# facebookresearch/detectron2

Hardware: NVIDIA H100
Metric: Mask R-CNN R50-FPN training hot-path images/sec (custom-op path fwd+bwd, 2 images/GPU) (higher is better)
Workload: dtype f32

## Files before the change

### detectron2_b200/csrc/deform_conv_tc.cu

```cuda
#include <algorithm>
#include <cstdlib>
#include <type_traits>

#include "common.cuh"
#include "deform_conv_tc.cuh"
#include "tc_common.cuh"

using namespace d2b_tc;

namespace {

constexpr int kWorkerWarps = 16;
constexpr int kWorkers = kWorkerWarps * 32;
constexpr int kThreads = kWorkers + 128;
constexpr int kLaunchRegs = (65536 / kThreads) & ~7;
constexpr int kWorkerRegs = 112, kSideRegs = 24;
static_assert(kWorkers * kWorkerRegs + (kThreads - kWorkers) * kSideRegs <= kThreads * kLaunchRegs,
              "register budget exceeds the launch allocation");
constexpr int kSideRegsMax = ((kThreads * kLaunchRegs - kWorkers * kWorkerRegs) / (kThreads - kWorkers)) & ~7;
static_assert(kSideRegsMax >= kSideRegs, "register budget exceeds the launch allocation");
constexpr int kMaxBN = 128;
constexpr int kRowsPerHalf = 128 / (2 * kWorkerWarps);
constexpr int kTile = 16384;
constexpr int kMaxSmem = 227 * 1024;
// ... 9 lines not shown
  long long off_bs, mask_bs;
  int mask_sigmoid;
};

struct Epi {
  const float* scale;
  const float* shift;
  int relu;
};

struct K1P { int BN, noct, goct, uper, ksplit, S, tap_bytes, stage_bytes, red; };
struct K2P { int mper, msplit, tap_bytes; };
struct K3P { int BN, noct, sper, nsplit, S, stage_bytes; };

inline size_t align256(size_t v) { return (v + 255) & ~(size_t)255; }

bool make_tc(const d2b_dcn_params* p, TC& d) {
  if (!p) return false;
  d.N = p->N; d.Cin = p->Cin; d.H = p->H; d.W = p->W; d.Cout = p->Cout; d.kh = p->kh; d.kw = p->kw;
  d.sh = p->stride_h; d.sw = p->stride_w; d.ph = p->pad_h; d.pw = p->pad_w; d.dh = p->dil_h; d.dw = p->dil_w;
  d.G = p->groups; d.DG = p->deformable_groups;
  if (d.N < 0 || d.Cin <= 0 || d.H <= 0 || d.W <= 0 || d.Cout <= 0 || d.kh <= 0 || d.kw <= 0 || d.sh <= 0 || d.sw <= 0 ||
      d.ph < 0 || d.pw < 0 || d.dh <= 0 || d.dw <= 0 || d.G <= 0 || d.DG <= 0)
    return false;
  if (d.Cin % d.G || d.Cout % d.G || d.Cin % d.DG) return false;
  d.Ho = (d.H + 2 * d.ph - (d.dh * (d.kh - 1) + 1)) / d.sh + 1;
  d.Wo = (d.W + 2 * d.pw - (d.dw * (d.kw - 1) + 1)) / d.sw + 1;
  if (d.Ho <= 0 || d.Wo <= 0) return false;
  d.cpg = d.Cin / d.G; d.opg = d.Cout / d.G; d.cpdg = d.Cin / d.DG; d.KK = d.kh * d.kw; d.HoWo = d.Ho * d.Wo;
  if (d.cpg >= 64) {
    if (d.cpg % 64) return false;
    d.pack = 1;
  } else {
    if (d.cpg != 16 && d.cpg != 32) return false;
    d.pack = 64 / d.cpg;
    if (d.G % d.pack) return false;
  }
  if (d.cpdg % 64) return false;
  d.SG = d.G / d.pack; d.cps = d.cpg * d.pack; d.ops = d.opg * d.pack; d.cbs = d.cps / 64; d.U = d.KK * d.cbs;
  if (d.ops % 16) return false;
  if (d.KK > 49) return false;
  if ((long long)d.H * d.W * d.Cin >= (1LL << 29)) return false;
  if ((long long)d.HoWo * d.Cout >= (1LL << 31) || (long long)d.Cout * d.cpg * d.KK >= (1LL << 31)) return false;
  d.tiles_img = d2b_cdiv(d.HoWo, 128);
  d.stages_img = d2b_cdiv(d.HoWo, 64);
  d.MC = (d.U + 1) / 2;
  d.nks = d.ops / 64;
  if ((long long)d.N * d.tiles_img > 0x7fffffffLL) return false;
  d.off_bs = (long long)d.DG * 2 * d.KK * d.HoWo;
  d.mask_bs = (long long)d.DG * d.KK * d.HoWo;
  d.mask_sigmoid = 0;
  return true;
}

const float* use_fused_offset_mask(TC& d, const float* offset_mask) {
  d.off_bs = d.mask_bs = (long long)d.DG * 3 * d.KK * d.HoWo;
  d.mask_sigmoid = 1;
  return offset_mask + (size_t)d.DG * 2 * d.KK * d.HoWo;
}

int largest_tile(int n) {
  for (int t = kMaxBN; t >= 16; t >>= 1)
    if (n % t == 0) return t;
  return 0;
}

int best_split(long long base, int work, int max_split, int overhead) {
  int best = 1;
  long long best_cost = -1;
  for (int s = 1; s <= max_split; ++s) {
    const int per = d2b_cdiv(work, s);
    const int parts = d2b_cdiv(work, per);
    const long long cost = (long long)d2b_cdiv(base * parts, d2b_num_sms()) * (per + overhead);
    if (best_cost < 0 || cost < best_cost) {
      best_cost = cost;
      best = parts;
    }
  }
  return best;
}

int k1_tap_points(const TC& d, int units) { return std::min(d.KK, (units + d.cbs - 2) / d.cbs + 1); }

bool plan_k1(const TC& d, K1P& k, bool colfed = false) {
  k.BN = largest_tile(d.ops);
  if (k.BN < 16) return false;
  k.noct = d.ops / k.BN;
  k.goct = colfed ? 1 : k.noct;
  const int base = d.N * d.tiles_img * d.SG * k.goct;
  k.ksplit = best_split(base, d.U, d.U, d.cbs);
  k.uper = d2b_cdiv(d.U, k.ksplit);
  k.ksplit = d2b_cdiv(d.U, k.uper);
  k.red = k.ksplit > 1;
  const int ndg = d.DG == 1 ? 1 : std::min(d.DG, d2b_cdiv(d.cps, d.cpdg) + 1);
  k.tap_bytes = ndg * k1_tap_points(d, k.uper) * 128 * 16;
  k.stage_bytes = 2 * kTile + 2 * k.BN * 128;
  k.S = 3;
  while (k.S > 1 && k.S * k.stage_bytes + k.tap_bytes + 1024 + 128 > kMaxSmem) --k.S;
  return k.S >= 2;
}

bool plan_k1c(const TC& d, K1P& k1, K1P& kc) {
  const long long base = (long long)d.N * d.tiles_img * d.SG * (k1.noct - 1);
  if (k1.goct != 1 || k1.noct < 2 || (long long)d.N * d.tiles_img * (k1.noct - 1) > 0x7fffffffLL) return false;
  kc = k1;
  kc.goct = k1.noct - 1;
  kc.ksplit = best_split(base, d.U, d.U, d.cbs);
  kc.uper = d2b_cdiv(d.U, kc.ksplit);
  kc.ksplit = d2b_cdiv(d.U, kc.uper);
  kc.tap_bytes = 0;
  kc.S = 3;
  while (kc.S > 1 && kc.S * kc.stage_bytes + 1024 + 128 > kMaxSmem) --kc.S;
  if (kc.S < 2) return false;
  k1.red = kc.red = k1.ksplit > 1 || kc.ksplit > 1;
  return true;
}

bool plan_k2(const TC& d, K2P& k) {
  if (d.ops % 64) return false;
  const int base = d.N * d.tiles_img * d.SG;
  k.msplit = best_split(base, d.MC, d.MC, 1);
  k.mper = d2b_cdiv(d.MC, k.msplit);
  k.msplit = d2b_cdiv(d.MC, k.mper);
  const int nkp = std::min(d.KK, (2 * k.mper + d.cbs - 1) / d.cbs + 1);
  const int ndg = d.DG == 1 ? 1 : std::min(d.DG, d2b_cdiv(d.cps, d.cpdg) + 1);
  k.tap_bytes = ndg * nkp * 128 * 16;
  return 2 * 4 * kTile + 128 * kGcolPitch * 4 + k.tap_bytes + 1024 + 128 <= kMaxSmem;
}

bool plan_k3(const TC& d, K3P& k) {
  if (d.ops % 64) return false;
  k.BN = largest_tile(d.ops);
  k.noct = d.ops / k.BN;
  const int units = d.MC * d.SG * k.noct;
  const int total = d.N * d.stages_img;
  k.nsplit = best_split(units, total, std::min(total, 4 * d2b_num_sms()), 3);
  k.sper = d2b_cdiv(total, k.nsplit);
  k.nsplit = d2b_cdiv(total, k.sper);
  k.stage_bytes = 2 * kTile + 2 * k.BN * 128;
  k.S = 3;
  while (k.S > 1 && k.S * k.stage_bytes + 4096 + 1024 + 128 > kMaxSmem) --k.S;
  return k.S >= 2;
}

struct Carve {
  size_t total = 0;
  size_t add(size_t bytes) {
    const size_t at = total;
    total += align256(bytes);
    return at;
  }
};

struct FwdPlan {
  TC d;
  K1P k1, kc;
  bool colfed;
  int split;
  size_t wt, x, total;
  size_t cols_bytes;
};

bool plan_fwd(const d2b_dcn_params* p, int precision, int x_nhwc, bool cols, FwdPlan& P) {
  if (!make_tc(p, P.d) || !plan_k1(P.d, P.k1)) return false;
  const TC& d = P.d;
  Carve ws;
  P.wt = ws.add((size_t)d.SG * P.k1.noct * d.U * 2 * P.k1.BN * 128);
  P.x = ws.add(x_nhwc ? 0 : sizeof(float) * (size_t)d.N * d.H * d.W * d.Cin);
  P.total = ws.total;
  P.cols_bytes = (size_t)d.N * d.tiles_img * d.SG * d.U * (size_t)(precision == 1 ? 2 : 1) * kTile;
  P.split = precision == 1 ? 1 : 0;
  P.colfed = false;
  K1P k1;
  if (cols && P.k1.noct > 1 && plan_k1(d, k1, true) && plan_k1c(d, k1, P.kc)) {
    P.k1 = k1;
    P.colfed = true;
  }
  return true;
}

struct BwdPlan {
  TC d;
  K2P k2;
  K3P k3;
  int split;
  size_t x, gx, gt_px, wt, gt_oc, gw, gw_bytes, total;
};

bool plan_bwd(const d2b_dcn_params* p, int precision, int x_nhwc, int need_data, int need_weight, BwdPlan& P) {
  if (!make_tc(p, P.d) || !plan_k2(P.d, P.k2) || !plan_k3(P.d, P.k3)) return false;
  const TC& d = P.d;
  const size_t xbytes = sizeof(float) * (size_t)d.N * d.H * d.W * d.Cin;
  P.gw_bytes = sizeof(float) * (size_t)d.SG * d.MC * 128 * d.ops;
  Carve ws;
  P.x = ws.add(x_nhwc ? 0 : xbytes);
  P.gx = ws.add(need_data && !x_nhwc ? xbytes : 0);
  P.gt_px = ws.add(need_data ? (size_t)d.N * d.tiles_img * d.SG * d.nks * 2 * kTile : 0);
  P.wt = ws.add(need_data ? (size_t)d.SG * d.MC * d.nks * 2 * kTile : 0);
  P.gt_oc = ws.add(need_weight ? (size_t)d.N * d.stages_img * d.SG * P.k3.noct * 2 * P.k3.BN * 128 : 0);
  P.gw = ws.add(need_weight ? P.gw_bytes : 0);
  P.total = ws.total;
  P.split = precision == 1 ? 1 : 0;
  return true;
}

struct TapRaw {
  float oh, ow, m;
};

__device__ __forceinline__ TapRaw tap_loads(const TC& d, const float* __restrict__ offset, const float* __restrict__ mask,
                                            int b, int dg, int kp, int p) {
  TapRaw r = {0.f, 0.f, 1.f};
  if (p < d.HoWo) {
    const size_t ob = (size_t)b * d.off_bs + ((size_t)dg * 2 * d.KK) * d.HoWo;
    r.oh = __ldg(offset + ob + (size_t)(2 * kp) * d.HoWo + p);
    r.ow = __ldg(offset + ob + (size_t)(2 * kp + 1) * d.HoWo + p);
    if (mask) r.m = __ldg(mask + (size_t)b * d.mask_bs + ((size_t)dg * d.KK + kp) * d.HoWo + p);
  }
  return r;
}

__device__ __forceinline__ int4 tap_finish(const TC& d, const TapRaw& r, bool has_mask, int kp, int p) {
  int4 t = make_int4(0, 0, 0, 0);
  if (p < d.HoWo) {
    const int ho = p / d.Wo, wo = p - ho * d.Wo;
    const int ki = kp / d.kw, kj = kp - ki * d.kw;
    const float hf = (float)(ho * d.sh - d.ph + ki * d.dh) + r.oh;
    const float wf = (float)(wo * d.sw - d.pw + kj * d.dw) + r.ow;
    float m = r.m;
    if (has_mask && d.mask_sigmoid) m = 1.f / (1.f + expf(-m));
    if (hf > -1.f && wf > -1.f && hf < (float)d.H && wf < (float)d.W) {
      const float hfl = floorf(hf), wfl = floorf(wf);
      const int hl = (int)hfl, wl = (int)wfl;
      const bool t0 = hl >= 0, t1 = hl + 1 <= d.H - 1, l0 = wl >= 0, l1 = wl + 1 <= d.W - 1;
      const int flags = (t0 && l0 ? 1 : 0) | (t0 && l1 ? 2 : 0) | (t1 && l0 ? 4 : 0) | (t1 && l1 ? 8 : 0);
      t.x = ((hl * d.W + wl + d.W + 1) << 4) | flags;
      t.y = __float_as_int(hf - hfl);
      t.z = __float_as_int(wf - wfl);
      t.w = __float_as_int(m);
    }
  }
  return t;
}

__device__ __forceinline__ int4 make_tap(const TC& d, const float* __restrict__ offset, const float* __restrict__ mask,
                                         int b, int dg, int kp, int p) {
  return tap_finish(d, tap_loads(d, offset, mask, b, dg, kp, p), mask != nullptr, kp, p);
}

struct Taps4 {
  float4 v0, v1, v2, v3;
};

__device__ __forceinline__ void load_corners(const float* __restrict__ xcb, uint32_t Cin, uint32_t rs, int code, Taps4& t) {
  const float* __restrict__ p = xcb + (uint32_t)(code >> 4) * Cin;
  const float4 z = make_float4(0.f, 0.f, 0.f, 0.f);
  t.v0 = (code & 1) ? __ldg(reinterpret_cast<const float4*>(p)) : z;
  t.v1 = (code & 2) ? __ldg(reinterpret_cast<const float4*>(p + Cin)) : z;
  t.v2 = (code & 4) ? __ldg(reinterpret_cast<const float4*>(p + rs)) : z;
  t.v3 = (code & 8) ? __ldg(reinterpret_cast<const float4*>(p + (rs + Cin))) : z;
}

__device__ __forceinline__ void interp4(const Taps4& t, float w0, float w1, float w2, float w3, float (&v)[4]) {
  const F2 z = f2_pack(0.f, 0.f), p0 = f2_pack(w0, w0), p1 = f2_pack(w1, w1), p2 = f2_pack(w2, w2), p3 = f2_pack(w3, w3);
  F2 a = f2_fma(p0, f2_pack(t.v0.x, t.v0.y), z), b = f2_fma(p0, f2_pack(t.v0.z, t.v0.w), z);
  a = f2_fma(p1, f2_pack(t.v1.x, t.v1.y), a);
  b = f2_fma(p1, f2_pack(t.v1.z, t.v1.w), b);
  a = f2_fma(p2, f2_pack(t.v2.x, t.v2.y), a);
  b = f2_fma(p2, f2_pack(t.v2.z, t.v2.w), b);
  a = f2_fma(p3, f2_pack(t.v3.x, t.v3.y), a);
  b = f2_fma(p3, f2_pack(t.v3.z, t.v3.w), b);
  f2_unpack(a, v[0], v[1]);
  f2_unpack(b, v[2], v[3]);
}

__device__ __forceinline__ void gather_store(const Taps4& t, int4 tap, uint8_t* a_hi, uint8_t* a_lo, uint32_t off,
                                             bool split) {
  const float lh = __int_as_float(tap.y), lw = __int_as_float(tap.z), m = __int_as_float(tap.w);
  const float hh = 1.f - lh, hw = 1.f - lw;
  float v[4];
  interp4(t, hh * hw * m, hh * lw * m, lh * hw * m, lh * lw * m, v);
  uint2 hi, lo;
  split4(v, hi, lo);
  *reinterpret_cast<uint2*>(a_hi + off) = hi;
  if (split) *reinterpret_cast<uint2*>(a_lo + off) = lo;
}

template <int BN, int kTransA, int kSplit>
__device__ __forceinline__ void mma_stage_(float (&acc)[BN / 4], uint32_t a_hi, uint32_t a_lo, uint32_t b_hi, uint32_t b_lo) {
  const int g = (threadIdx.x >> 7);
  const uint32_t ao = kTransA ? (uint32_t)(g & 1) * 8192u : (uint32_t)(g & 1) * 64u * 128u;
  const uint32_t bo = (uint32_t)(g >> 1) * (uint32_t)(BN / 2) * 128u;
  const uint32_t lbo = kTransA ? 8192u : 0u;
  wgmma_fence();
#pragma unroll
  for (int kk = 0; kk < 4; ++kk) {
    const uint32_t ak = ao + (kTransA ? (uint32_t)kk * 2048u : (uint32_t)kk * 32u), bk = bo + (uint32_t)kk * 32u;
    Wgmma<BN / 2, kTransA>::mma(acc, wgmma_desc(a_hi + ak, lbo, 1024), wgmma_desc(b_hi + bk, 0, 1024), 1);
    if (kSplit) {
      Wgmma<BN / 2, kTransA>::mma(acc, wgmma_desc(a_hi + ak, lbo, 1024), wgmma_desc(b_lo + bk, 0, 1024), 1);
      Wgmma<BN / 2, kTransA>::mma(acc, wgmma_desc(a_lo + ak, lbo, 1024), wgmma_desc(b_hi + bk, 0, 1024), 1);
    }
  }
  wgmma_commit();
}
template <int BN, int kTransA>
__device__ __forceinline__ void mma_stage(float (&acc)[BN / 4], uint32_t a_hi, uint32_t a_lo, uint32_t b_hi, uint32_t b_lo,
                                          int split) {
  if (split) mma_stage_<BN, kTransA, 1>(acc, a_hi, a_lo, b_hi, b_lo);
  else mma_stage_<BN, kTransA, 0>(acc, a_hi, a_lo, b_hi, b_lo);
}

template <int BN>
__device__ __forceinline__ int acc_row(int i) {
  const int t = threadIdx.x & 127;
  return (threadIdx.x >> 7 & 1) * 64 + (t >> 5) * 16 + ((t & 31) >> 2) + ((i >> 1) & 1) * 8;
}
template <int BN>
__device__ __forceinline__ int acc_col(int i) {
  return (threadIdx.x >> 8) * (BN / 2) + (i >> 2) * 8 + (threadIdx.x & 3) * 2 + (i & 1);
}

template <int BN>
__device__ __forceinline__ void fwd_epilogue(const float (&acc)[BN / 4], const Epi& ep, const TC& d, const K1P& k,
                                             float* __restrict__ out, int b, int p0, int oc0) {
  const bool add_shift = ep.shift != nullptr && blockIdx.z == 0;
#pragma unroll
  for (int i = 0; i < BN / 4; ++i) {
    const int p = p0 + acc_row<BN>(i);
    if (p >= d.HoWo) continue;
    const int oc = oc0 + acc_col<BN>(i);
    float* dst = out + ((size_t)b * d.Cout + oc) * d.HoWo + p;
    float v = acc[i];
    if (k.red) {
      red_add(dst, v + ((add_shift && !ep.scale && !ep.relu) ? __ldg(ep.shift + oc) : 0.f));
    } else {
      if (ep.scale) v *= __ldg(ep.scale + oc);
      if (ep.shift) v += __ldg(ep.shift + oc);
      if (ep.relu) v = fmaxf(v, 0.f);
      *dst = v;
    }
  }
}

template <int BN>
__global__ void __launch_bounds__(kThreads, 1) dcn_fwd_tc_kernel(const float* __restrict__ xh,
                                                                   const float* __restrict__ offset,
                                                                   const float* __restrict__ mask,
                                                                   const uint8_t* __restrict__ wt, const Epi ep, const TC d,
                                                                   const K1P k, const int split, float* __restrict__ out,
                                                                   uint8_t* __restrict__ cols) {
// ... 548 lines not shown
      if (have_next && lane < 2 * PX)
        my_taps[((i + 1) & 1) * (2 * PX) + lane] =
            tl_ok ? tap_finish(d, raw, mask != nullptr, tl_kp, pbn + warp * PX + tl_j) : make_int4(0, 0, 0, 0);
      fence_proxy_async();
      __syncwarp();
      if (lane == 0) mbar_arrive(&full_bar[s]);
      mbar_wait(&full_bar[s], par);
      const uint32_t sa = smem_u32(smem + s * k.stage_bytes), sb = sa + 2 * kTile;
      mma_stage<BN, 1>(acc, sa, sa + kTile, sb, sb + (uint32_t)BN * 128u, split);
    };
    stage(0);
    for (int i = 1; i < ns; ++i) {
      stage(i);
      wgmma_wait<1>();
      __syncwarp();
      if (lane == 0) mbar_arrive(&empty_bar[(i - 1) % k.S]);
    }
    wgmma_wait<0>();
    gw_tile_store<BN>(acc, gw + ((size_t)sg * d.MC * 128 + (size_t)mb * 128) * d.ops + (size_t)oct * k.BN, d.ops);
  } else if (warp == kWorkerWarps) {
    if (lane == 0) {
      const uint32_t bytes = (uint32_t)(split ? 2 : 1) * (uint32_t)k.BN * 128u;
      for (int i = 0; i < ns; ++i) {
        const int s = i % k.S;
        const uint32_t par = (uint32_t)((i / k.S) & 1);
        mbar_wait(&empty_bar[s], par ^ 1u);
        mbar_arrive_expect_tx(&full_bar[s], bytes);
        const size_t tile = ((size_t)(gs0 + i) * d.SG + sg) * k.noct + oct;
        bulk_g2s(smem + s * k.stage_bytes + 2 * kTile, gt + tile * (size_t)(2 * k.BN * 128), bytes, &full_bar[s]);
      }
    }
  }
}

template <int BN, int kSide>
__device__ __forceinline__ void bwd_weight_cols_body(uint8_t* smem, int bx, int by, int bz, const uint8_t* __restrict__ cols,
                                                     const uint8_t* __restrict__ gt, const TC& d, const K3P& k, const int S,
                                                     const int split, float* __restrict__ gw) {
  uint64_t* bars = reinterpret_cast<uint64_t*>(smem + S * k.stage_bytes);
  uint64_t* full_bar = bars;
  uint64_t* empty_bar = bars + S;

  const int tid = threadIdx.x, warp = tid >> 5, lane = tid & 31;
  const int mb = by;
  const int sg = bx / k.noct, oct = bx - sg * k.noct;
  const int total = d.N * d.stages_img;
  const int gs0 = bz * k.sper, gs1 = min(total, gs0 + k.sper), ns = gs1 - gs0;
  const int nu = (2 * mb + 1 < d.U) ? 2 : 1;

  if (tid == 0) {
    for (int s = 0; s < S; ++s) {
      mbar_init(&full_bar[s], 1);
      mbar_init(&empty_bar[s], kWorkerWarps);
    }
    mbar_init_fence();
  }
  if (nu == 1 && tid < kWorkers) {
    for (int s = 0; s < S; ++s)
      for (int i = tid; i < 2 * 512; i += kWorkers) {
        const int part = i >> 9, w = i & 511;
        reinterpret_cast<uint4*>(smem + s * k.stage_bytes + part * kTile + 8192)[w] = make_uint4(0, 0, 0, 0);
      }
    fence_proxy_async();
  }
  __syncthreads();
  if (warp < kWorkerWarps) reg_alloc<kWorkerRegs>();
  else reg_dealloc<kSide>();

  if (warp < kWorkerWarps) {
    float acc[BN / 4];
#pragma unroll
    for (int i = 0; i < BN / 4; ++i) acc[i] = 0.f;
    auto issue = [&](int i) {
      const int s = i % S;
      mbar_wait(&full_bar[s], (uint32_t)((i / S) & 1));
      const uint32_t sa = smem_u32(smem + s * k.stage_bytes), sb = sa + 2 * kTile;
      mma_stage<BN, 1>(acc, sa, sa + kTile, sb, sb + (uint32_t)BN * 128u, split);
    };
    issue(0);
    for (int i = 1; i < ns; ++i) {
      issue(i);
      wgmma_wait<1>();
      __syncwarp();
      if (lane == 0) mbar_arrive(&empty_bar[(i - 1) % S]);
    }
    wgmma_wait<0>();
    gw_tile_store<BN>(acc, gw + ((size_t)sg * d.MC * 128 + (size_t)mb * 128) * d.ops + (size_t)oct * k.BN, d.ops);
  } else if (warp == kWorkerWarps) {
    if (lane == 0) {
      const uint32_t parts = split ? 2u : 1u;
      const uint32_t tile_bytes = parts * (uint32_t)kTile;
      const uint32_t gbytes = parts * (uint32_t)k.BN * 128u;
      for (int i = 0; i < ns; ++i) {
        const int s = i % S;
        const uint32_t par = (uint32_t)((i / S) & 1);
        const int gs = gs0 + i;
        const int b = gs / d.stages_img, st = gs - b * d.stages_img;
        mbar_wait(&empty_bar[s], par ^ 1u);
        mbar_arrive_expect_tx(&full_bar[s], (uint32_t)nu * parts * 8192u + gbytes);
        uint8_t* stage = smem + s * k.stage_bytes;
        const uint8_t* src =
            cols + ((((size_t)b * d.tiles_img + (st >> 1)) * d.SG + sg) * d.U + 2 * mb) * tile_bytes + (size_t)(st & 1) * 8192;
        for (int ul = 0; ul < nu; ++ul)
          for (uint32_t part = 0; part < parts; ++part)
            bulk_g2s(stage + part * kTile + ul * 8192, src + (size_t)ul * tile_bytes + (size_t)part * kTile, 8192u, &full_bar[s]);
        const size_t tile = ((size_t)gs * d.SG + sg) * k.noct + oct;
        bulk_g2s(stage + 2 * kTile, gt + tile * (size_t)(2 * k.BN * 128), gbytes, &full_bar[s]);
      }
    }
  }
}

template <int BN>
__global__ void __launch_bounds__(kThreads, 1) dcn_bwd_weight_cols_kernel(const uint8_t* __restrict__ cols,
                                                                          const uint8_t* __restrict__ gt, const TC d,
                                                                          const K3P k, const int S, const int split,
                                                                          float* __restrict__ gw) {
  bwd_weight_cols_body<BN, kSideRegs>(aligned_smem(), blockIdx.x, blockIdx.y, blockIdx.z, cols, gt, d, k, S, split, gw);
}

template <int BN>
__global__ void __launch_bounds__(kThreads, 1) dcn_bwd_fused_kernel(const float* __restrict__ xh,
                                                                    const float* __restrict__ offset,
                                                                    const float* __restrict__ mask,
                                                                    const uint8_t* __restrict__ gt_px,
                                                                    const uint8_t* __restrict__ wt, const K2P k2,
                                                                    float* __restrict__ gxh, float* __restrict__ goff,
                                                                    float* __restrict__ gmask,
                                                                    const uint8_t* __restrict__ cols,
                                                                    const uint8_t* __restrict__ gt_oc, const K3P k3,
                                                                    const int S3, float* __restrict__ gw, const TC d,
                                                                    const int split) {
  const int nx2 = d.N * d.tiles_img, n2 = nx2 * d.SG * k2.msplit;
  int id = blockIdx.x;
  if (id < n2) {
    const int bx = id % nx2, r = id / nx2;
    bwd_data_body<kSideRegsMax>(aligned_smem(), bx, r % d.SG, r / d.SG, xh, offset, mask, gt_px, wt, d, k2, split, gxh, goff,
                                gmask);
  } else {
    id -= n2;
    const int nx3 = d.SG * k3.noct, r = id / nx3;
    bwd_weight_cols_body<BN, kSideRegsMax>(aligned_smem(), id % nx3, r % d.MC, r / d.MC, cols, gt_oc, d, k3, S3, split,
                                           gw);
  }
}

__device__ __forceinline__ void split8(const float (&v)[8], uint4& hi, uint4& lo) {
  split2(v[0], v[1], hi.x, lo.x);
  split2(v[2], v[3], hi.y, lo.y);
  split2(v[4], v[5], hi.z, lo.z);
  split2(v[6], v[7], hi.w, lo.w);
}

__device__ __forceinline__ float w_elem(const float* __restrict__ w, const TC& d, int oc, int c, int kp) {
  const int g = c / d.cpg;
  if (oc / d.opg != g) return 0.f;
  return __ldg(w + ((size_t)oc * d.cpg + (c - g * d.cpg)) * d.KK + kp);
}

__global__ void dcn_wtile_fwd_kernel(const float* __restrict__ w, const TC d, int BN, int noct, uint8_t* __restrict__ dst) {
  const long long idx = (long long)blockIdx.x * blockDim.x + threadIdx.x;
  const long long total = (long long)d.SG * noct * d.U * BN * 8;
  if (idx >= total) return;
  const int c16 = (int)(idx & 7);
  const int r = (int)((idx >> 3) % BN);
  const long long tile = idx / (8LL * BN);
  const int u = (int)(tile % d.U);
  const int oct = (int)((tile / d.U) % noct);
  const int sg = (int)(tile / ((long long)d.U * noct));
  const int kp = u / d.cbs, cb = u - kp * d.cbs;
  const int oc = sg * d.ops + oct * BN + r;
  float v[8];
#pragma unroll
  for (int e = 0; e < 8; ++e) v[e] = w_elem(w, d, oc, sg * d.cps + cb * 64 + c16 * 8 + e, kp);
  uint4 hi, lo;
  split8(v, hi, lo);
  uint8_t* base = dst + tile * (size_t)(2 * BN * 128);
  *reinterpret_cast<uint4*>(base + swz128((uint32_t)r, (uint32_t)c16)) = hi;
  *reinterpret_cast<uint4*>(base + BN * 128 + swz128((uint32_t)r, (uint32_t)c16)) = lo;
}

__global__ void dcn_wtile_bwd_kernel(const float* __restrict__ w, const TC d, uint8_t* __restrict__ dst) {
  const long long idx = (long long)blockIdx.x * blockDim.x + threadIdx.x;
  const long long total = (long long)d.SG * d.MC * d.nks * 128 * 8;
  if (idx >= total) return;
  const int c16 = (int)(idx & 7);
  const int r = (int)((idx >> 3) & 127);
  const long long tile = idx >> 10;
  const int ks = (int)(tile % d.nks);
  const int m = (int)((tile / d.nks) % d.MC);
  const int sg = (int)(tile / ((long long)d.nks * d.MC));
  const int u = 2 * m + (r >> 6);
  float v[8];
#pragma unroll
  for (int e = 0; e < 8; ++e) v[e] = 0.f;
  if (u < d.U) {
    const int kp = u / d.cbs, cb = u - kp * d.cbs;
    const int c = sg * d.cps + cb * 64 + (r & 63);
#pragma unroll
    for (int e = 0; e < 8; ++e) v[e] = w_elem(w, d, sg * d.ops + ks * 64 + c16 * 8 + e, c, kp);
  }
  uint4 hi, lo;
  split8(v, hi, lo);
  uint8_t* base = dst + tile * (size_t)(2 * kTile);
  *reinterpret_cast<uint4*>(base + swz128((uint32_t)r, (uint32_t)c16)) = hi;
  *reinterpret_cast<uint4*>(base + kTile + swz128((uint32_t)r, (uint32_t)c16)) = lo;
}

__device__ __forceinline__ float gout_elem(const float* __restrict__ gout, const float* __restrict__ ysaved, const Epi& ep,
                                           size_t idx, int oc) {
  float g = __ldg(gout + idx);
  if (ep.relu && !(__ldg(ysaved + idx) > 0.f)) g = 0.f;
  if (ep.scale) g *= __ldg(ep.scale + oc);
  return g;
}

__global__ void __launch_bounds__(256) dcn_gout_px_tiles_kernel(const float* __restrict__ gout,
                                                                const float* __restrict__ ysaved, const Epi ep, const TC d,
                                                                uint8_t* __restrict__ dst, uint8_t* __restrict__ dst_oc,
                                                                int BN, int noct) {
  __shared__ float t[64][33];
  const long long tile = blockIdx.x;
  const int ks = (int)(tile % d.nks);
  const int sg = (int)((tile / d.nks) % d.SG);
  const int pt = (int)((tile / ((long long)d.nks * d.SG)) % d.tiles_img);
  const int b = (int)(tile / ((long long)d.nks * d.SG * d.tiles_img));
  const int r0 = blockIdx.y * 32;
  const int p0 = pt * 128 + r0, oc0 = sg * d.ops + ks * 64;
  const int tid = threadIdx.x;
#pragma unroll
  for (int i = 0; i < 8; ++i) {
    const int e = tid + i * 256;
    const int o = e >> 5, pp = e & 31;
    const int p = p0 + pp;
    t[o][pp] = p < d.HoWo ? gout_elem(gout, ysaved, ep, ((size_t)b * d.Cout + oc0 + o) * d.HoWo + p, oc0 + o) : 0.f;
  }
  __syncthreads();
  uint8_t* base = dst + tile * (size_t)(2 * kTile);
  {
    const int r = tid >> 3, c16 = tid & 7;
    float v[8];
#pragma unroll
    for (int i = 0; i < 8; ++i) v[i] = t[c16 * 8 + i][r];
    uint4 hi, lo;
    split8(v, hi, lo);
    *reinterpret_cast<uint4*>(base + swz128((uint32_t)(r0 + r), (uint32_t)c16)) = hi;
    *reinterpret_cast<uint4*>(base + kTile + swz128((uint32_t)(r0 + r), (uint32_t)c16)) = lo;
  }
  if (dst_oc) {
    const int o = tid >> 2, ch = tid & 3;
    const int ocs = ks * 64 + o;
    const int oct = ocs / BN, row = ocs - oct * BN;
    const int pglob = pt * 128 + r0;
    const int ps = pglob >> 6, c16 = ((pglob & 63) >> 3) + ch;
    float v[8];
#pragma unroll
    for (int i = 0; i < 8; ++i) v[i] = t[o][ch * 8 + i];
    uint4 hi, lo;
    split8(v, hi, lo);
    if (ps < d.stages_img) {
      const size_t tile_oc = (((size_t)b * d.stages_img + ps) * d.SG + sg) * noct + oct;
      uint8_t* bo = dst_oc + tile_oc * (size_t)(2 * BN * 128);
      *reinterpret_cast<uint4*>(bo + swz128((uint32_t)row, (uint32_t)c16)) = hi;
      *reinterpret_cast<uint4*>(bo + BN * 128 + swz128((uint32_t)row, (uint32_t)c16)) = lo;
    }
  }
}

__global__ void dcn_gout_oc_tiles_kernel(const float* __restrict__ gout, const float* __restrict__ ysaved, const Epi ep,
                                         const TC d, int BN, int noct, uint8_t* __restrict__ dst) {
  const long long idx = (long long)blockIdx.x * blockDim.x + threadIdx.x;
  const long long total = (long long)d.N * d.stages_img * d.SG * noct * BN * 8;
  if (idx >= total) return;
  const int c16 = (int)(idx & 7);
  const int r = (int)((idx >> 3) % BN);
  const long long tile = idx / (8LL * BN);
  const int oct = (int)(tile % noct);
  const int sg = (int)((tile / noct) % d.SG);
  const int ps = (int)((tile / ((long long)noct * d.SG)) % d.stages_img);
  const int b = (int)(tile / ((long long)noct * d.SG * d.stages_img));
  const int oc = sg * d.ops + oct * BN + r;
  const size_t src = ((size_t)b * d.Cout + oc) * d.HoWo;
  float v[8];
#pragma unroll
  for (int e = 0; e < 8; ++e) {
    const int p = ps * 64 + c16 * 8 + e;
    v[e] = p < d.HoWo ? gout_elem(gout, ysaved, ep, src + p, oc) : 0.f;
  }
  uint4 hi, lo;
  split8(v, hi, lo);
  uint8_t* base = dst + tile * (size_t)(2 * BN * 128);
  *reinterpret_cast<uint4*>(base + swz128((uint32_t)r, (uint32_t)c16)) = hi;
  *reinterpret_cast<uint4*>(base + BN * 128 + swz128((uint32_t)r, (uint32_t)c16)) = lo;
}

__global__ void dcn_epilogue_kernel(float* __restrict__ y, long long total, int Cout, int HoWo, const Epi ep) {
  const long long i = (long long)blockIdx.x * blockDim.x + threadIdx.x;
  if (i >= total) return;
  const int oc = (int)((i / HoWo) % Cout);
  float v = y[i];
  if (ep.scale) v *= __ldg(ep.scale + oc);
  if (ep.shift) v += __ldg(ep.shift + oc);
  if (ep.relu) v = fmaxf(v, 0.f);
  y[i] = v;
}

int change_layout(const float* src, const TC& d, float* dst, bool to_nhwc, cudaStream_t stream) {
  d2b_pyramid P = {};
  P.num_levels = 1;
  P.feat[0] = src;
  P.H[0] = d.H;
  P.W[0] = d.W;
  P.scale[0] = 1.f;
  float* dsts[1] = {dst};
  return to_nhwc ? d2b_pyramid_nchw_to_nhwc(&P, d.N, d.Cin, dsts, D2B_F32, (void*)stream)
                 : d2b_pyramid_nhwc_to_nchw(&P, d.N, d.Cin, reinterpret_cast<void* const*>(dsts), D2B_F32, (void*)stream);
}

template <auto kernel, class... Args>
int launch_big_smem(dim3 grid, int smem_bytes, cudaStream_t stream, Args... args) {
  D2B_ALLOW_BIG_SMEM(kernel);
  kernel<<<grid, kThreads, smem_bytes, stream>>>(args...);
  D2B_CHECK_LAUNCH();
  return D2B_OK;
}

template <int W, int... More, class Launch>
int with_tile_width(int BN, Launch launch) {
  if constexpr (sizeof...(More) > 0)
    if (BN != W) return with_tile_width<More...>(BN, launch);
  return launch(std::integral_constant<int, W>());
}

}

D2B_API int d2b_deform_conv_tc_shape_supported(const d2b_dcn_params* p, int backward) {
  FwdPlan f;
  BwdPlan b;
  return backward ? plan_bwd(p, 1, 1, 1, 1, b) : plan_fwd(p, 1, 1, false, f);
}

size_t d2b_deform_conv_tc_fwd_workspace(const d2b_dcn_params* p, int precision, int x_nhwc) {
  FwdPlan P;
  return plan_fwd(p, precision, x_nhwc, false, P) ? P.total : 0;
}

size_t d2b_deform_conv_tc_bwd_workspace(const d2b_dcn_params* p, int precision, int x_nhwc, int need_data, int need_weight) {
  BwdPlan P;
  return plan_bwd(p, precision, x_nhwc, need_data, need_weight, P) ? P.total : 0;
}

size_t d2b_deform_conv_tc_cols_bytes(const d2b_dcn_params* p, int precision) {
  FwdPlan f;
  BwdPlan b;
  return plan_fwd(p, precision, 1, false, f) && plan_bwd(p, precision, 1, 0, 0, b) ? f.cols_bytes : 0;
}

int d2b_deform_conv_forward_tc(const float* x, const float* offset, const float* mask, const float* weight,
                               const float* scale, const float* shift, int relu, const d2b_dcn_params* p, int precision,
                               int tcflags, float* out, void* cols, void* workspace, size_t workspace_bytes, void* stream_) {
  cudaStream_t stream = (cudaStream_t)stream_;
  const int x_nhwc = tcflags & 1;
  FwdPlan P;
  if (!plan_fwd(p, precision, x_nhwc, cols != nullptr, P)) return D2B_EUNSUPPORTED;
  TC& d = P.d;
  const K1P& k = P.k1;
  if (d.N == 0) return D2B_OK;
  if (tcflags & 2) {
    if (mask) return D2B_EINVAL;
    mask = use_fused_offset_mask(d, offset);
  }
  if (!workspace || workspace_bytes < P.total) return D2B_EWORKSPACE;
  if ((reinterpret_cast<uintptr_t>(workspace) & 255) || (x_nhwc && (reinterpret_cast<uintptr_t>(x) & 15)) ||
      (reinterpret_cast<uintptr_t>(cols) & 15))
    return D2B_EINVAL;
  uint8_t* ws = reinterpret_cast<uint8_t*>(workspace);
  uint8_t* wt = ws + P.wt;
  const float* xh = x;
  if (!x_nhwc) {
    float* xn = reinterpret_cast<float*>(ws + P.x);
    if (int rc = change_layout(x, d, xn, true, stream)) return rc;
    xh = xn;
  }
  {
    const long long total = (long long)d.SG * k.noct * d.U * k.BN * 8;
    dcn_wtile_fwd_kernel<<<d2b_cdiv(total, 256), 256, 0, stream>>>(weight, d, k.BN, k.noct, wt);
    D2B_CHECK_LAUNCH();
  }
  if (k.red) D2B_CUDA(cudaMemsetAsync(out, 0, sizeof(float) * (size_t)d.N * d.Cout * d.HoWo, stream));
  const Epi ep = {scale, shift, relu};
  const dim3 grid(d.N * d.tiles_img, d.SG * k.goct, k.ksplit);
  const int smem_bytes = k.S * k.stage_bytes + k.tap_bytes + 1024 + 128;
  int rc = with_tile_width<16, 32, 64, 128>(k.BN, [&](auto bn) {
    return launch_big_smem<dcn_fwd_tc_kernel<decltype(bn)::value>>(grid, smem_bytes, stream, xh, offset, mask, wt, ep, d, k,
                                                                    P.split, out, reinterpret_cast<uint8_t*>(cols));
  });
  if (rc) return rc;
  if (P.colfed) {
    const K1P& kc = P.kc;
    const dim3 grid_c(d.N * d.tiles_img * kc.goct, d.SG, kc.ksplit);
    const int smem_c = kc.S * kc.stage_bytes + 1024 + 128;
    const uint8_t* cl = reinterpret_cast<const uint8_t*>(cols);
    rc = with_tile_width<16, 32, 64, 128>(kc.BN, [&](auto bn) {
      return launch_big_smem<dcn_fwd_cols_kernel<decltype(bn)::value>>(grid_c, smem_c, stream, cl, wt, ep, d, kc, P.split,
                                                                        out);
    });
    if (rc) return rc;
  }
  if (k.red && (scale || relu)) {
    const long long total = (long long)d.N * d.Cout * d.HoWo;
    dcn_epilogue_kernel<<<d2b_cdiv(total, 256), 256, 0, stream>>>(out, total, d.Cout, d.HoWo, ep);
    D2B_CHECK_LAUNCH();
  }
  return D2B_OK;
}

int d2b_deform_conv_backward_tc(const float* x, const float* offset, const float* mask, const float* weight,
                                const float* grad_out, const float* scale, const float* y_saved, int relu,
                                const d2b_dcn_params* p, int precision, int tcflags, const void* cols, float* grad_x,
                                float* grad_offset, float* grad_mask, float* grad_weight, void* workspace,
                                size_t workspace_bytes, void* stream_) {
  cudaStream_t stream = (cudaStream_t)stream_;
  const int x_nhwc = tcflags & 1;
  const int need_data = (grad_x || grad_offset || grad_mask) ? 1 : 0, need_weight = grad_weight ? 1 : 0;
  BwdPlan P;
  if (!plan_bwd(p, precision, x_nhwc, need_data, need_weight, P)) return D2B_EUNSUPPORTED;
  TC& d = P.d;
  const K2P& k2 = P.k2;
  const K3P& k3 = P.k3;
  const bool fused_om = (tcflags & 2) != 0;
  if (fused_om && (mask || grad_mask)) return D2B_EINVAL;
  if (relu && !y_saved) return D2B_EINVAL;
  const size_t nx = (size_t)d.N * d.H * d.W * d.Cin, noff = (size_t)d.N * d.DG * (fused_om ? 3 : 2) * d.KK * d.HoWo;
  const size_t nm = (size_t)d.N * d.DG * d.KK * d.HoWo, nw = (size_t)d.Cout * d.cpg * d.KK;
  if (fused_om) {
    mask = use_fused_offset_mask(d, offset);
    if (grad_offset) grad_mask = grad_offset + (size_t)d.DG * 2 * d.KK * d.HoWo;
  }
  const Epi ep = {scale, nullptr, relu};
  if (d.N == 0 || (!need_data && !need_weight)) {
    void* zp[3] = {grad_offset, fused_om ? nullptr : grad_mask, grad_weight};
    size_t zb[3] = {noff * 4, nm * 4, nw * 4};
    return d2b_zero_buffers(zp, zb, 3, stream);
  }
  if (!workspace || workspace_bytes < P.total) return D2B_EWORKSPACE;
  if ((reinterpret_cast<uintptr_t>(workspace) & 255) || (x_nhwc && (reinterpret_cast<uintptr_t>(x) & 15)) ||
      (x_nhwc && grad_x && (reinterpret_cast<uintptr_t>(grad_x) & 15)) || (reinterpret_cast<uintptr_t>(cols) & 15))
    return D2B_EINVAL;
  uint8_t* ws = reinterpret_cast<uint8_t*>(workspace);
  const float* xh = x;
  if (!x_nhwc) {
    float* xn = reinterpret_cast<float*>(ws + P.x);
    if (int rc = change_layout(x, d, xn, true, stream)) return rc;
    xh = xn;
  }
  float* gxh = grad_x ? (x_nhwc ? grad_x : reinterpret_cast<float*>(ws + P.gx)) : nullptr;
  uint8_t* gt_oc = need_weight ? ws + P.gt_oc : nullptr;
  float* gw_part = need_weight ? reinterpret_cast<float*>(ws + P.gw) : nullptr;
  {
    void* zp[4] = {grad_offset, fused_om ? nullptr : grad_mask, gxh, gw_part};
    size_t zb[4] = {noff * 4, nm * 4, nx * 4, P.gw_bytes};
    int rc = d2b_zero_buffers(zp, zb, 4, stream);
    if (rc) return rc;
  }
  const long long fused_ctas = (long long)d.N * d.tiles_img * d.SG * k2.msplit + (long long)d.SG * k3.noct * d.MC * k3.nsplit;
  const bool fused = need_data && need_weight && cols && fused_ctas <= 0x7fffffffLL;
  const uint8_t* cl = reinterpret_cast<const uint8_t*>(cols);
  const int S3 = std::min(6, (kMaxSmem - 2048) / k3.stage_bytes);
  const int smem3 = S3 * k3.stage_bytes + 1024 + 128;
  if (need_data) {
    uint8_t* gt_px = ws + P.gt_px;
    uint8_t* wt = ws + P.wt;
    dcn_gout_px_tiles_kernel<<<dim3((unsigned)((size_t)d.N * d.tiles_img * d.SG * d.nks), 4), 256, 0, stream>>>(
        grad_out, y_saved, ep, d, gt_px, gt_oc, k3.BN, k3.noct);
    D2B_CHECK_LAUNCH();
    {
      const long long total = (long long)d.SG * d.MC * d.nks * 128 * 8;
      dcn_wtile_bwd_kernel<<<d2b_cdiv(total, 256), 256, 0, stream>>>(weight, d, wt);
      D2B_CHECK_LAUNCH();
    }
    const int smem2 = 2 * 4 * kTile + 128 * kGcolPitch * 4 + k2.tap_bytes + 1024 + 128;
    float* gm = mask ? grad_mask : nullptr;
    int rc;
    if (fused) {
      rc = with_tile_width<64, 128>(k3.BN, [&](auto bn) {
        return launch_big_smem<dcn_bwd_fused_kernel<decltype(bn)::value>>(
            dim3((unsigned)fused_ctas), std::max(smem2, smem3), stream, xh, offset, mask, gt_px, wt, k2, gxh, grad_offset, gm,
            cl, gt_oc, k3, S3, gw_part, d, P.split);
      });
    } else {
      rc = launch_big_smem<dcn_bwd_data_tc_kernel>(dim3(d.N * d.tiles_img, d.SG, k2.msplit), smem2, stream, xh, offset, mask,
                                                   gt_px, wt, d, k2, P.split, gxh, grad_offset, gm);
    }
    if (rc) return rc;
    if (grad_x && !x_nhwc) {
      if (int rc = change_layout(gxh, d, grad_x, false, stream)) return rc;
    }
  }
  if (need_weight) {
    if (!need_data) {
      const long long total = (long long)d.N * d.stages_img * d.SG * k3.noct * k3.BN * 8;
      dcn_gout_oc_tiles_kernel<<<d2b_cdiv(total, 256), 256, 0, stream>>>(grad_out, y_saved, ep, d, k3.BN, k3.noct, gt_oc);
      D2B_CHECK_LAUNCH();
    }
    if (!fused) {
      const dim3 grid(d.SG * k3.noct, d.MC, k3.nsplit);
      int rc;
      if (cols) {
        rc = with_tile_width<64, 128>(k3.BN, [&](auto bn) {
          return launch_big_smem<dcn_bwd_weight_cols_kernel<decltype(bn)::value>>(grid, smem3, stream, cl, gt_oc, d, k3, S3,
                                                                                   P.split, gw_part);
        });
      } else {
        const int smem_bytes = k3.S * k3.stage_bytes + 4096 + 1024 + 128;
        rc = with_tile_width<64, 128>(k3.BN, [&](auto bn) {
          return launch_big_smem<dcn_bwd_weight_tc_kernel<decltype(bn)::value>>(grid, smem_bytes, stream, xh, offset, mask,
                                                                                 gt_oc, d, k3, P.split, gw_part);
        });
      }
      if (rc) return rc;
    }
    if (d.KK <= 9) {
      dcn_gw_reduce_tile_kernel<<<dim3(d.SG * (d.cps / kRedCh), d.ops / kRedOc), 256, 0, stream>>>(gw_part, d, grad_weight);
    } else {
      const long long total = (long long)d.SG * d.U * 64 * d.ops;
      dcn_gw_reduce_kernel<<<d2b_cdiv(total, 256), 256, 0, stream>>>(gw_part, d, grad_weight);
    }
    D2B_CHECK_LAUNCH();
  }
  return D2B_OK;
}
```

Baseline: 300.3.

## Build fwd and bwd DCN weight tiles in one smem-staged kernel, reuse in backward

Replaces the two per-element weight-tiling kernels with one kernel that stages a block of weights in shared memory using vectorized loads and writes both forward and backward swizzled tiles. The backward tile is stored after the saved columns buffer during forward, so backward skips rebuilding it when columns are available. This cuts global-load redundancy and one launch per backward, at the cost of a larger saved columns buffer. It also assumes ops divisible by 16/64 and KK<=49, which can break for other shapes.

```diff
diff --git a/detectron2_b200/csrc/deform_conv_tc.cu b/detectron2_b200/csrc/deform_conv_tc.cu
--- a/detectron2_b200/csrc/deform_conv_tc.cu
+++ b/detectron2_b200/csrc/deform_conv_tc.cu
@@ -185,13 +185,18 @@
   }
 };
 
+size_t wt_bwd_bytes(const TC& d) { return (size_t)d.SG * d.MC * d.nks * 2 * kTile; }
+size_t cols_wt_offset(const TC& d, int precision) {
+  return ((size_t)d.N * d.tiles_img * d.SG * d.U * (size_t)(precision == 1 ? 2 : 1) * kTile + 1023) & ~(size_t)1023;
+}
+
 struct FwdPlan {
   TC d;
   K1P k1, kc;
   bool colfed;
   int split;
   size_t wt, x, total;
-  size_t cols_bytes;
+  size_t cols_wt, cols_bytes;
 };
 
 bool plan_fwd(const d2b_dcn_params* p, int precision, int x_nhwc, bool cols, FwdPlan& P) {
@@ -201,7 +206,8 @@
   P.wt = ws.add((size_t)d.SG * P.k1.noct * d.U * 2 * P.k1.BN * 128);
   P.x = ws.add(x_nhwc ? 0 : sizeof(float) * (size_t)d.N * d.H * d.W * d.Cin);
   P.total = ws.total;
-  P.cols_bytes = (size_t)d.N * d.tiles_img * d.SG * d.U * (size_t)(precision == 1 ? 2 : 1) * kTile;
+  P.cols_wt = cols_wt_offset(d, precision);
+  P.cols_bytes = P.cols_wt + (d.ops % 64 == 0 ? wt_bwd_bytes(d) : 0);
   P.split = precision == 1 ? 1 : 0;
   P.colfed = false;
   K1P k1;
@@ -229,7 +235,7 @@
   P.x = ws.add(x_nhwc ? 0 : xbytes);
   P.gx = ws.add(need_data && !x_nhwc ? xbytes : 0);
   P.gt_px = ws.add(need_data ? (size_t)d.N * d.tiles_img * d.SG * d.nks * 2 * kTile : 0);
-  P.wt = ws.add(need_data ? (size_t)d.SG * d.MC * d.nks * 2 * kTile : 0);
+  P.wt = ws.add(need_data ? wt_bwd_bytes(d) : 0);
   P.gt_oc = ws.add(need_weight ? (size_t)d.N * d.stages_img * d.SG * P.k3.noct * 2 * P.k3.BN * 128 : 0);
   P.gw = ws.add(need_weight ? P.gw_bytes : 0);
   P.total = ws.total;
@@ -1084,59 +1090,83 @@
   split2(v[6], v[7], hi.w, lo.w);
 }
 
-__device__ __forceinline__ float w_elem(const float* __restrict__ w, const TC& d, int oc, int c, int kp) {
-  const int g = c / d.cpg;
-  if (oc / d.opg != g) return 0.f;
-  return __ldg(w + ((size_t)oc * d.cpg + (c - g * d.cpg)) * d.KK + kp);
-}
-
-__global__ void dcn_wtile_fwd_kernel(const float* __restrict__ w, const TC d, int BN, int noct, uint8_t* __restrict__ dst) {
-  const long long idx = (long long)blockIdx.x * blockDim.x + threadIdx.x;
-  const long long total = (long long)d.SG * noct * d.U * BN * 8;
-  if (idx >= total) return;
-  const int c16 = (int)(idx & 7);
-  const int r = (int)((idx >> 3) % BN);
-  const long long tile = idx / (8LL * BN);
-  const int u = (int)(tile % d.U);
-  const int oct = (int)((tile / d.U) % noct);
-  const int sg = (int)(tile / ((long long)d.U * noct));
-  const int kp = u / d.cbs, cb = u - kp * d.cbs;
-  const int oc = sg * d.ops + oct * BN + r;
-  float v[8];
-#pragma unroll
-  for (int e = 0; e < 8; ++e) v[e] = w_elem(w, d, oc, sg * d.cps + cb * 64 + c16 * 8 + e, kp);
-  uint4 hi, lo;
-  split8(v, hi, lo);
-  uint8_t* base = dst + tile * (size_t)(2 * BN * 128);
-  *reinterpret_cast<uint4*>(base + swz128((uint32_t)r, (uint32_t)c16)) = hi;
-  *reinterpret_cast<uint4*>(base + BN * 128 + swz128((uint32_t)r, (uint32_t)c16)) = lo;
-}
-
-__global__ void dcn_wtile_bwd_kernel(const float* __restrict__ w, const TC d, uint8_t* __restrict__ dst) {
-  const long long idx = (long long)blockIdx.x * blockDim.x + threadIdx.x;
-  const long long total = (long long)d.SG * d.MC * d.nks * 128 * 8;
-  if (idx >= total) return;
-  const int c16 = (int)(idx & 7);
-  const int r = (int)((idx >> 3) & 127);
-  const long long tile = idx >> 10;
-  const int ks = (int)(tile % d.nks);
-  const int m = (int)((tile / d.nks) % d.MC);
-  const int sg = (int)(tile / ((long long)d.nks * d.MC));
-  const int u = 2 * m + (r >> 6);
-  float v[8];
-#pragma unroll
-  for (int e = 0; e < 8; ++e) v[e] = 0.f;
-  if (u < d.U) {
-    const int kp = u / d.cbs, cb = u - kp * d.cbs;
-    const int c = sg * d.cps + cb * 64 + (r & 63);
-#pragma unroll
-    for (int e = 0; e < 8; ++e) v[e] = w_elem(w, d, sg * d.ops + ks * 64 + c16 * 8 + e, c, kp);
-  }
-  uint4 hi, lo;
-  split8(v, hi, lo);
-  uint8_t* base = dst + tile * (size_t)(2 * kTile);
-  *reinterpret_cast<uint4*>(base + swz128((uint32_t)r, (uint32_t)c16)) = hi;
-  *reinterpret_cast<uint4*>(base + kTile + swz128((uint32_t)r, (uint32_t)c16)) = lo;
+constexpr int kWtOc = 16;
+
+__global__ void __launch_bounds__(128) dcn_wtiles_kernel(const float* __restrict__ w, const TC d, int BN, int noct,
+                                                         uint8_t* __restrict__ fwd, uint8_t* __restrict__ bwd) {
+  __shared__ float s[kWtOc * (8 * 49 + 1)];
+  const int P = 8 * d.KK + 1;
+  const int nob = d.ops / kWtOc;
+  const int sg = blockIdx.x / nob, o0 = (blockIdx.x - sg * nob) * kWtOc;
+  const int c0 = blockIdx.y * 8;
+  const int cg = c0 / d.cpg;
+  const int tid = threadIdx.x;
+  {
+    const int n = 8 * d.KK;
+    const bool vec = (reinterpret_cast<uintptr_t>(w) & 15) == 0;
+    for (int r = tid >> 5; r < kWtOc; r += 4) {
+      const int oc = sg * d.ops + o0 + r;
+      float* sr = s + r * P;
+      if ((sg * d.pack + cg) * d.opg > oc || oc >= (sg * d.pack + cg + 1) * d.opg) {
+        for (int i = tid & 31; i < n; i += 32) sr[i] = 0.f;
+        continue;
+      }
+      const float* __restrict__ src = w + ((size_t)oc * d.cpg + (c0 - cg * d.cpg)) * d.KK;
+      if (vec) {
+        for (int i = tid & 31; i < n / 4; i += 32) {
+          const float4 v = __ldg(reinterpret_cast<const float4*>(src) + i);
+          sr[4 * i] = v.x;
+          sr[4 * i + 1] = v.y;
+          sr[4 * i + 2] = v.z;
+          sr[4 * i + 3] = v.w;
+        }
+      } else {
+        for (int i = tid & 31; i < n; i += 32) sr[i] = __ldg(src + i);
+      }
+    }
+  }
+  __syncthreads();
+  const int cb = c0 >> 6, c16 = (c0 & 63) >> 3;
+  if (fwd) {
+    const int oct = o0 / BN;
+    for (int i = tid; i < kWtOc * d.KK; i += 128) {
+      const int r = i % kWtOc, kp = i / kWtOc;
+      float v[8];
+#pragma unroll
+      for (int e = 0; e < 8; ++e) v[e] = s[r * P + e * d.KK + kp];
+      uint4 hi, lo;
+      split8(v, hi, lo);
+      const uint32_t row = (uint32_t)(o0 - oct * BN + r);
+      uint8_t* base = fwd + ((size_t)(sg * noct + oct) * d.U + kp * d.cbs + cb) * (size_t)(2 * BN * 128);
+      *reinterpret_cast<uint4*>(base + swz128(row, (uint32_t)c16)) = hi;
+      *reinterpret_cast<uint4*>(base + BN * 128 + swz128(row, (uint32_t)c16)) = lo;
+    }
+  }
+  if (bwd) {
+    const int ks = o0 >> 6;
+    for (int i = tid; i < 16 * d.KK; i += 128) {
+      const int cl = i & 7, h = (i >> 3) & 1, kp = i >> 4;
+      float v[8];
+#pragma unroll
+      for (int e = 0; e < 8; ++e) v[e] = s[(h * 8 + e) * P + cl * d.KK + kp];
+      uint4 hi, lo;
+      split8(v, hi, lo);
+      const int u = kp * d.cbs + cb, m = u >> 1;
+      const uint32_t row = (uint32_t)((u & 1) * 64 + (c0 & 63) + cl), chunk = (uint32_t)(((o0 & 63) >> 3) + h);
+      uint8_t* base = bwd + ((size_t)(sg * d.MC + m) * d.nks + ks) * (size_t)(2 * kTile);
+      *reinterpret_cast<uint4*>(base + swz128(row, chunk)) = hi;
+      *reinterpret_cast<uint4*>(base + kTile + swz128(row, chunk)) = lo;
+      if (u + 1 == d.U && !(u & 1)) {
+        const uint4 z = make_uint4(0u, 0u, 0u, 0u);
+        *reinterpret_cast<uint4*>(base + swz128(row + 64u, chunk)) = z;
+        *reinterpret_cast<uint4*>(base + kTile + swz128(row + 64u, chunk)) = z;
+      }
+    }
+  }
+}
+
+inline void launch_wtiles(const float* w, const TC& d, int BN, int noct, uint8_t* fwd, uint8_t* bwd, cudaStream_t stream) {
+  dcn_wtiles_kernel<<<dim3(d.SG * (d.ops / kWtOc), d.cps / 8), 128, 0, stream>>>(w, d, BN, noct, fwd, bwd);
 }
 
 __device__ __forceinline__ float gout_elem(const float* __restrict__ gout, const float* __restrict__ ysaved, const Epi& ep,
@@ -1314,11 +1344,9 @@
     if (int rc = change_layout(x, d, xn, true, stream)) return rc;
     xh = xn;
   }
-  {
-    const long long total = (long long)d.SG * k.noct * d.U * k.BN * 8;
-    dcn_wtile_fwd_kernel<<<d2b_cdiv(total, 256), 256, 0, stream>>>(weight, d, k.BN, k.noct, wt);
-    D2B_CHECK_LAUNCH();
-  }
+  launch_wtiles(weight, d, k.BN, k.noct, wt,
+                cols && d.ops % 64 == 0 ? reinterpret_cast<uint8_t*>(cols) + P.cols_wt : nullptr, stream);
+  D2B_CHECK_LAUNCH();
   if (k.red) D2B_CUDA(cudaMemsetAsync(out, 0, sizeof(float) * (size_t)d.N * d.Cout * d.HoWo, stream));
   const Epi ep = {scale, shift, relu};
   const dim3 grid(d.N * d.tiles_img, d.SG * k.goct, k.ksplit);
@@ -1402,13 +1430,12 @@
   const int smem3 = S3 * k3.stage_bytes + 1024 + 128;
   if (need_data) {
     uint8_t* gt_px = ws + P.gt_px;
-    uint8_t* wt = ws + P.wt;
     dcn_gout_px_tiles_kernel<<<dim3((unsigned)((size_t)d.N * d.tiles_img * d.SG * d.nks), 4), 256, 0, stream>>>(
         grad_out, y_saved, ep, d, gt_px, gt_oc, k3.BN, k3.noct);
     D2B_CHECK_LAUNCH();
-    {
-      const long long total = (long long)d.SG * d.MC * d.nks * 128 * 8;
-      dcn_wtile_bwd_kernel<<<d2b_cdiv(total, 256), 256, 0, stream>>>(weight, d, wt);
+    const uint8_t* wt = cl ? cl + cols_wt_offset(d, precision) : ws + P.wt;
+    if (!cl) {
+      launch_wtiles(weight, d, 0, 0, nullptr, ws + P.wt, stream);
       D2B_CHECK_LAUNCH();
     }
     const int smem2 = 2 * 4 * kTile + 128 * kGcolPitch * 4 + k2.tap_bytes + 1024 + 128;
```

Result: faster. 304.3, median of 6 (+1.3%).
